# Lapis-Hong/wide_deep

Hardware: NVIDIA B200
Metric: CTR examples/sec (train step) (higher is better)
Workload: dtype bf16x3 (fp32 operands split into bf16 hi+lo, 3 tensor-core products, fp32 accumulate; 2^-16)

## Files before the change

### wide_deep_b200/csrc/api.cu

```cuda
#include <stdarg.h>
#include <stdlib.h>
#include <string.h>

#include <algorithm>
#include <cmath>
#include <random>

#include "common.cuh"
#include "farmhash.cuh"
#include "sparse_dev.cuh"

namespace wd {
static thread_local char g_err[1024] = "";
void set_error(const char* fmt, ...) {
    va_list ap;
    va_start(ap, fmt);
    vsnprintf(g_err, sizeof(g_err), fmt, ap);
    va_end(ap);
}
int init_sparse_tables(WdModel* m, uint64_t seed, int random_w);
int dense_refresh_transposes(WdModel* m);
int wide_bias_grad(WdModel* m);
int metrics_setup();
int merge_sparse(WdModel* m, int which, const void* rows, const void* grads, int64_t n);
// ... 69 lines not shown
extern "C" uint64_t wd_fingerprint_cat64(uint64_t a, uint64_t b) { return wd::fingerprint_cat64(a, b); }

namespace wd { void tc_map_cache_clear(); }

extern "C" int wd_model_destroy(WdModel* m) {
    if (!m) return WD_OK;
    cudaSetDevice(m->device);
    if (m->stream) cudaStreamSynchronize(m->stream);
    tc_map_cache_clear();
    for (auto& sl : m->slots) {
        if (sl.graph) cudaGraphExecDestroy(sl.graph);
        if (sl.graph_bwd) cudaGraphExecDestroy(sl.graph_bwd);
        if (sl.ev_up) cudaEventDestroy(sl.ev_up);
        if (sl.ev_used) cudaEventDestroy(sl.ev_used);
    }
    if (m->stream_up) { cudaStreamSynchronize(m->stream_up); cudaStreamDestroy(m->stream_up); }
    for (auto& g : m->merge_graph) if (g.exec) cudaGraphExecDestroy(g.exec);
    if (m->ev_bwd_done) cudaEventDestroy(m->ev_bwd_done);
    for (void* p : m->allocs) cudaFree(p);
    if (m->h_loss_pinned) cudaFreeHost(m->h_loss_pinned);
    for (auto& e : m->timer.ev) if (e) cudaEventDestroy(e);
    if (m->shard.aux) { cudaStreamSynchronize(m->shard.aux); cudaStreamDestroy(m->shard.aux); }
    for (cudaEvent_t ev : {m->shard.ev_a, m->shard.ev_ids2, m->shard.ev_routed1, m->shard.ev_a2, m->shard.ev_aux_done}) if (ev) cudaEventDestroy(ev);
    for (int w = 0; w < 2; ++w) {
        if (m->sstream[w]) { cudaStreamSynchronize(m->sstream[w]); cudaStreamDestroy(m->sstream[w]); }
        if (m->ev_grouped[w]) cudaEventDestroy(m->ev_grouped[w]);
        if (m->ev_done[w]) cudaEventDestroy(m->ev_done[w]);
    }
    if (m->ev_ids) cudaEventDestroy(m->ev_ids);
    if (m->ev_wide_fwd) cudaEventDestroy(m->ev_wide_fwd);
    if (m->ev_wgrad_rest) cudaEventDestroy(m->ev_wgrad_rest);
    if (m->ev_head) cudaEventDestroy(m->ev_head);
    if (m->ev_dx0) cudaEventDestroy(m->ev_dx0);
    if (m->stream) cudaStreamDestroy(m->stream);
    for (size_t i = 0; i < g_extra.size(); ++i)
        if (g_extra[i].first == m) { delete g_extra[i].second; g_extra.erase(g_extra.begin() + i); break; }
    delete m;
    return WD_OK;
}

static int init_dense_slots(WdModel* m) {
    if (m->dense_count == 0) return WD_OK;
    std::vector<float> S1(m->dense_count, 0.f);
    for (size_t i = 0; i < m->dense.size(); ++i) {
        const WdOptimizer& o = (m->use_wide && i == 0) ? m->lin_opt : m->dnn_opt;
        float s1 = slot1_init(o);
        int64_t end = i + 1 < m->dense.size() ? m->dense[i + 1].off : m->dense_count;
        for (int64_t j = m->dense[i].off; j < end; ++j) S1[j] = s1;
    }
    WD_CUDA(cudaMemcpyAsync(m->d_S1, S1.data(), S1.size() * 4, cudaMemcpyHostToDevice, m->stream));
    WD_CUDA(cudaStreamSynchronize(m->stream));
    return WD_OK;
}

static int build_model(const WdPlanDesc* d, WdModel* m, WdModelExtra* x) {
    int rc;
    m->use_wide = d->model_type & 1;
    m->use_deep = (d->model_type & 2) != 0;
    m->n_cat_fields = d->n_cat_fields; m->n_dense_fields = d->n_dense_fields; m->n_columns = d->n_columns;
    const int C = d->n_columns;
    m->col_kind.assign(d->col_kind, d->col_kind + C);
    m->col_field.assign(d->col_field, d->col_field + C);
    m->col_buckets.assign(d->col_buckets, d->col_buckets + C);
    m->col_wide_base.assign(d->col_wide_base, d->col_wide_base + C);
    m->col_emb_table.assign(d->col_emb_table, d->col_emb_table + C);
    m->col_ind_off.assign(d->col_ind_off, d->col_ind_off + C);
// ... 211 lines not shown

        int hu_off = 0, did = 0;
        for (int t = 0; t < d->n_towers; ++t) {
            Tower tw{};
            tw.n_hidden = d->tower_nlayers[t]; tw.mode = d->tower_mode[t];
            std::vector<int> hu(d->hidden_units + hu_off, d->hidden_units + hu_off + tw.n_hidden);
            hu_off += tw.n_hidden;
            const std::vector<int> units = hu;
            if (m->crelu) for (int& h : hu) h *= 2;
            auto srcs = layer_sources(tw.mode, tw.n_hidden);
            for (int l = 0; l <= tw.n_hidden; ++l) {
                Layer L{};
                if ((int)srcs[l].size() > kMaxSegs) { set_error("layer with more than %d concatenated inputs", kMaxSegs); return WD_EUNSUPPORTED; }
                L.n_in_segs = (int)srcs[l].size();
                int koff = 0, klog = 0;
                for (int s = 0; s < L.n_in_segs; ++s) {
                    int src = srcs[l][s];
                    Seg sg{};
                    sg.src = src;
                    sg.width = src < 0 ? x->d0_logical : hu[src];
                    sg.width_phys = src < 0 ? d->d0_phys : pad_to(hu[src], 32);
                    sg.k_off = koff;
                    koff += sg.width_phys; klog += sg.width;
                    L.segs[s] = sg;
                }
                L.K = klog; L.K_phys = koff;
                const bool hidden = l < tw.n_hidden;
                L.N = hidden ? hu[l] : 1;
                L.N_phys = hidden ? pad_to(hu[l], 32) : 1;
                L.N_param = hidden ? units[l] : 1;
                L.t_gamma = L.t_beta = -1;
                L.h_fp32 = false;
                for (int src : srcs[tw.n_hidden]) if (src == l) L.h_fp32 = true;
                std::vector<int> idx(4, -1);
                if (hidden) {
                    {
                        const int tn = (m->gemm_engine == WD_GEMM_BF16X3 && L.N_phys % 256 == 0) ? 256 : 128;
                        const int tiles = ((L.K_phys + 127) / 128) * ((L.N_phys + tn - 1) / tn);
                        int sp = m->wgrad_splits;
                        while (sp < 32 && tiles * sp * 2 <= 148 && m->max_batch_pad / (sp * 2) >= 512) sp *= 2;
                        L.wgrad_splits = sp;
                    }
                    L.t_kernel = add_dense(L.K_phys, L.N_phys, L.wgrad_splits, 0, (int64_t)L.K_phys * L.N_phys, true);
                    L.t_bias = add_dense(1, L.N_phys, m->row_tiles, 1, L.N_phys, false);
                    if (m->crelu) m->dense[L.t_kernel].mirror_u = m->dense[L.t_bias].mirror_u = L.N_param;
                    if (m->batch_norm) {
                        L.t_gamma = add_dense(1, L.N_phys, m->row_tiles, 1, L.N_phys, false);
                        L.t_beta = add_dense(1, L.N_phys, m->row_tiles, 1, L.N_phys, false);
                    }
                    const int64_t n = (int64_t)m->max_batch_pad * L.N_phys;
                    if ((rc = dev_alloc(m, &L.H, n))) return rc;
                    if (m->batch_norm || m->dropout_rate > 0.f) { if ((rc = dev_alloc(m, &L.A, n))) return rc; } else L.A = L.H;
                    if ((rc = dev_alloc(m, &L.HT, n))) return rc;
                    if ((rc = dev_alloc(m, &L.dH, n))) return rc;
                    if ((rc = dev_alloc(m, &L.dZ, n))) return rc;
                    if ((rc = dev_alloc(m, &L.dZT, n))) return rc;
                    if (m->gemm_engine == WD_GEMM_BF16X3)
                        for (int part = 0; part < 2; ++part) {
                            if ((rc = dev_alloc(m, &L.Hs[part], n))) return rc;
                            if ((rc = dev_alloc(m, &L.dZs[part], n))) return rc;
                        }
                } else {
                    L.t_kernel = add_dense(L.K_phys, 1, m->row_tiles, 1, L.K_phys, false);
                    L.t_bias = add_dense(1, 1, m->row_tiles, 1, 4, false);
                }
                idx[WD_D_KERNEL] = L.t_kernel; idx[WD_D_BIAS] = L.t_bias; idx[WD_D_GAMMA] = L.t_gamma; idx[WD_D_BETA] = L.t_beta;
// ... 67 lines not shown
    for (auto& e : m->timer.ev) WD_CUDA(cudaEventCreate(&e));
    WD_CUDA(cudaStreamSynchronize(m->stream));
    return WD_OK;
}

extern "C" int wd_model_create(const WdPlanDesc* d, int device, WdModel** out) {
    if (!d || !out) { set_error("null argument"); return WD_EINVAL; }
    if (d->api_version != WD_API_VERSION) { set_error("plan api_version %d != library %d", d->api_version, WD_API_VERSION); return WD_EINVAL; }
    int ndev = 0;
    if (cudaGetDeviceCount(&ndev) != cudaSuccess || ndev == 0) {
        set_error("no CUDA device: libwd_b200 has no CPU fallback");
        return WD_ENODEVICE;
    }
    if (device < 0 || device >= ndev) { set_error("device %d out of range (%d devices)", device, ndev); return WD_EINVAL; }
    WD_CUDA(cudaSetDevice(device));
    WdModel* m = new WdModel();
    WdModelExtra* x = new WdModelExtra();
    g_extra.push_back({m, x});
    m->device = device;
    memset(m->timer.ev, 0, sizeof(m->timer.ev));
    cudaError_t e = cudaStreamCreateWithFlags(&m->stream, cudaStreamNonBlocking);
    if (e == cudaSuccess) e = cudaStreamCreateWithFlags(&m->stream_up, cudaStreamNonBlocking);
    for (int w = 0; w < 2; ++w) {
        if (e == cudaSuccess) e = cudaStreamCreateWithFlags(&m->sstream[w], cudaStreamNonBlocking);
        if (e == cudaSuccess) e = cudaEventCreateWithFlags(&m->ev_grouped[w], cudaEventDisableTiming);
        if (e == cudaSuccess) e = cudaEventCreateWithFlags(&m->ev_done[w], cudaEventDisableTiming);
    }
    if (e == cudaSuccess) e = cudaEventCreateWithFlags(&m->ev_ids, cudaEventDisableTiming);
    if (e == cudaSuccess) e = cudaEventCreateWithFlags(&m->ev_wide_fwd, cudaEventDisableTiming);
    if (e == cudaSuccess) e = cudaEventCreateWithFlags(&m->ev_wgrad_rest, cudaEventDisableTiming);
    if (e == cudaSuccess) e = cudaEventCreateWithFlags(&m->ev_head, cudaEventDisableTiming);
    if (e == cudaSuccess) e = cudaEventCreateWithFlags(&m->ev_dx0, cudaEventDisableTiming);
    if (e == cudaSuccess) e = cudaEventCreateWithFlags(&m->ev_bwd_done, cudaEventDisableTiming);
    if (e != cudaSuccess) { set_error("cudaStreamCreate: %s", cudaGetErrorString(e)); wd_model_destroy(m); return WD_ECUDA; }
    m->graphs_enabled = getenv("WD_NO_GRAPH") == nullptr;
    int rc = build_model(d, m, x);
    if (rc) { wd_model_destroy(m); return rc; }
    *out = m;
    return WD_OK;
}

static int init_dense(WdModel* m, WdModelExtra* x, uint64_t seed) {
    if (m->dense_count == 0) return WD_OK;
    std::vector<float> P(m->dense_count, 0.f), S1(m->dense_count, 0.f), S2(m->dense_count, 0.f);
    std::mt19937_64 rng(seed * 7919 + 17);
    std::uniform_real_distribution<float> U(-1.f, 1.f);
    for (size_t ti = 0; ti < m->towers.size(); ++ti) {
        Tower& tw = m->towers[ti];
        for (int l = 0; l <= tw.n_hidden; ++l) {
            Layer& L = tw.layers[l];
            const DenseTensor& tk = m->dense[L.t_kernel];
            const float lim = std::sqrt(6.f / (float)(L.K + L.N_param));
            for (int s = 0; s < L.n_in_segs; ++s) {
                const Seg& sg = L.segs[s];
                for (int j = 0; j < sg.width_phys; ++j) {
                    bool real = sg.src < 0 ? (x->x0_real[j] != 0) : (j < sg.width);
                    if (!real) continue;
                    float* prow = &P[tk.off + (int64_t)(sg.k_off + j) * L.N_phys];
                    for (int n = 0; n < L.N_param; ++n) {
                        prow[n] = lim * U(rng);
                        if (tk.mirror_u) prow[n + tk.mirror_u] = -prow[n];
                    }
                }
            }
            if (L.t_gamma >= 0) for (int n = 0; n < L.N; ++n) P[m->dense[L.t_gamma].off + n] = 1.f;
        }
// ... 893 lines not shown
```

### wide_deep_b200/csrc/common.cuh

```cuda
#pragma once
#include <cuda_bf16.h>
#include <cuda_runtime.h>
#include <stdint.h>
#include <stdio.h>
#include <string>
#include <vector>

#include "../../include/wd_b200.h"

namespace wd {

constexpr int kSortTile = 1024;

void set_error(const char* fmt, ...);

#define WD_CUDA(call)                                                                         \
    do {                                                                                      \
        cudaError_t e__ = (call);                                                             \
        if (e__ != cudaSuccess) {                                                             \
            wd::set_error("%s:%d %s -> %s", __FILE__, __LINE__, #call, cudaGetErrorString(e__)); \
            return WD_ECUDA;                                                                  \
        }                                                                                     \
    } while (0)

// ... 62 lines not shown
    int64_t count;
    int rows, cols;
    int64_t gpart_off;
    int gparts;
    int g_rowtiles;
    int64_t gstride;
    int64_t wt_off;
    int mirror_u;
};

struct Seg {
    int src;
    int width;
    int width_phys;
    int k_off;
};

struct Layer {
    int n_in_segs;
    Seg segs[kMaxSegs];
    int K, K_phys;
    int N, N_phys;
    int N_param;
    int t_kernel, t_bias, t_gamma, t_beta;
    int wgrad_splits;
    float* A;
    float* H;
    float* HT;
    float* dH;
    float* dZ;
    float* dZT;
    __nv_bfloat16 *Hs[2], *dZs[2];
    bool h_fp32;
    float* colpart;
};

struct Tower {
    int n_hidden;
    int mode;
    std::vector<Layer> layers;
    float* logit;
};

struct PhaseTimer {
    static constexpr int kMax = 160;
    cudaEvent_t ev[kMax];
    const char* name[kMax];
    float ms[kMax];
    int n = 0, n_last = 0;
    bool enabled = false;
};

struct BatchSlot {
    int32_t* off = nullptr;
    uint64_t* keys = nullptr;
    float *dense = nullptr, *label = nullptr, *weight = nullptr;
    DevBatch view{};
    bool has_label = false, filled = false;
    cudaEvent_t ev_up = nullptr;
    cudaEvent_t ev_used = nullptr;
    bool up_pending = false, used_recorded = false;
    cudaGraphExec_t graph = nullptr;
    DevBatch graph_view{};
    int64_t graph_launches = 0;
    int eager_steps = 0;
    cudaGraphExec_t graph_bwd = nullptr;
// ... 55 lines not shown
    uint64_t step = 0;
    cudaEvent_t ev_a = nullptr;
    cudaStream_t aux = nullptr;
    cudaEvent_t ev_ids2 = nullptr, ev_routed1 = nullptr, ev_a2 = nullptr, ev_aux_done = nullptr;
    cudaGraphExec_t graph[64] = {};
    DevBatch graph_view[64];
    int64_t graph_launches[64] = {};
    int eager_steps[64] = {};
};
constexpr int kBarriers = 8;

}

struct WdModel {
    int device = 0;
    bool use_wide = false, use_deep = false;
    int n_cat_fields = 0, n_dense_fields = 0, n_columns = 0;
    std::vector<int32_t> col_kind, col_field, col_aux_off, col_aux_n, col_norm_kind, col_emb_table, col_ind_off;
    std::vector<int64_t> col_buckets, col_wide_base;
    std::vector<float> col_norm_a, col_norm_b;
    int n_numeric = 0;
    int d0_phys = 0;
    int64_t wide_rows = 0;
    int activation = 0, batch_norm = 0;
    WdOptimizer lin_opt{}, dnn_opt{};
    int max_batch = 0, max_batch_pad = 0;
    int64_t max_nnz = 0;
    int gemm_engine = 0;

    cudaStream_t stream = nullptr;
    cudaStream_t sstream[2] = {nullptr, nullptr};
    cudaStream_t stream_up = nullptr;
    cudaEvent_t ev_ids = nullptr, ev_head = nullptr, ev_dx0 = nullptr, ev_bwd_done = nullptr, ev_wide_fwd = nullptr, ev_wgrad_rest = nullptr;
    bool sort_smem_opt_in = false;
    bool crelu = false;
    bool list_apply_fused[2] = {false, false};
    bool record_wgrad_rest = false;
    int dense_split_tensor = -1, dense_part = 0;
    cudaEvent_t ev_grouped[2] = {nullptr, nullptr}, ev_done[2] = {nullptr, nullptr};
    bool side_pending[2] = {false, false};
    bool side_active[2] = {false, false};
    bool record_dx0 = false, dx0_recorded = false;
    struct MergeGraph { cudaGraphExec_t exec = nullptr; const void* rows = nullptr; const void* grads = nullptr; int64_t n = 0; int n_lists = 0;
                        bool on_side = false; int eager = 0; int64_t launches = 0; } merge_graph[2];
    int64_t dense_exchange_max_rows = 0;
    int64_t small_base[2] = {0, 0};
    int64_t gs_count = 0, gs_emb_floats = 0;
    int64_t gs_touch_off[2] = {0, 0};
    int n_rtab = 0, n_small_tab = 0;
    int64_t* d_rtab_row_base = nullptr;
    float** d_rtab_data = nullptr;
    int32_t *d_rtab_dim = nullptr, *d_rtab_stride = nullptr;
    int64_t* d_rtab_gs_off = nullptr;
    int32_t* d_nubig[2] = {nullptr, nullptr};
    wd::ShardState shard;
    wd::DevPlan dplan{};
    std::vector<void*> allocs;
    int64_t bytes_allocated = 0;

    int32_t *d_num_field = nullptr, *d_num_norm_kind = nullptr, *d_num_x0_off = nullptr;
    float *d_num_a = nullptr, *d_num_b = nullptr;

    int32_t* d_cat_offsets = nullptr;
    uint64_t* d_cat_keys = nullptr;
    int64_t keys_cap = 0;
    float *d_dense = nullptr, *d_label = nullptr, *d_weight = nullptr;
// ... 153 lines not shown
```

### wide_deep_b200/csrc/gemm_bf16.cu

```cuda
#include <cuda.h>
#include <stdlib.h>

#include "common.cuh"
#include "gemm.cuh"
#include "tc_ptx.cuh"

namespace wd {

int tc_make_map_bf16(CUtensorMap* map, const void* ptr, int rows, int cols, int ld, int box_rows);

namespace {

__device__ __forceinline__ void sts128(uint32_t a, uint32_t x, uint32_t y, uint32_t z, uint32_t w) {
    asm volatile("st.shared.v4.b32 [%0], {%1, %2, %3, %4};" ::"r"(a), "r"(x), "r"(y), "r"(z), "r"(w) : "memory");
}
__device__ __forceinline__ uint4 lds128(uint32_t a) {
    uint4 v;
    asm volatile("ld.shared.v4.b32 {%0, %1, %2, %3}, [%4];" : "=r"(v.x), "=r"(v.y), "=r"(v.z), "=r"(v.w) : "r"(a) : "memory");
    return v;
}
__device__ __forceinline__ void sts32f(uint32_t a, float x) { asm volatile("st.shared.f32 [%0], %1;" ::"r"(a), "f"(x) : "memory"); }
__device__ __forceinline__ float4 lds128f(uint32_t a) {
    float4 v;
    asm volatile("ld.shared.v4.f32 {%0, %1, %2, %3}, [%4];" : "=f"(v.x), "=f"(v.y), "=f"(v.z), "=f"(v.w) : "r"(a) : "memory");
// ... 244 lines not shown
                            v[4 * j4] = __float_as_uint(a0); v[4 * j4 + 1] = __float_as_uint(a1); v[4 * j4 + 2] = __float_as_uint(a2); v[4 * j4 + 3] = __float_as_uint(a3);
                            h[4 * j4] = __float_as_uint(fmaf(a0, g4.x, e4.x)); h[4 * j4 + 1] = __float_as_uint(fmaf(a1, g4.y, e4.y));
                            h[4 * j4 + 2] = __float_as_uint(fmaf(a2, g4.z, e4.z)); h[4 * j4 + 3] = __float_as_uint(fmaf(a3, g4.w, e4.w));
                        }
                        if (nb + 32 > ep.n_logical) {
#pragma unroll
                            for (int j = 0; j < 32; ++j) if (nb + j >= ep.n_logical) { v[j] = 0u; h[j] = 0u; }
                        }
                    } else {
#pragma unroll
                        for (int j = 0; j < 32; ++j) {
                            const bool ok = (nb + j) < ep.n_logical;
                            const float av = ok ? act_fwd(ep.act, __uint_as_float(v[j]) + lds32f(wp + 4 * j)) : 0.f;
                            v[j] = __float_as_uint(av);
                            h[j] = __float_as_uint(ok ? fmaf(av, lds32f(wp + 4 * (32 + j)), lds32f(wp + 4 * (64 + j))) : 0.f);
                        }
                    }
                    if (!rv) {
#pragma unroll
                        for (int j = 0; j < 32; ++j) { v[j] = 0u; h[j] = 0u; }
                    }
                    if (ep.A_out != ep.H_out) store_f32(ep.A_out, ep.ldh, mw, nb, v, false);
                    if (ep.H_out) store_f32(ep.H_out, ep.ldh, mw, nb, h, false);
                    uint32_t hh[16], hl[16];
#pragma unroll
                    for (int j = 0; j < 16; ++j) {
                        const float x0 = __uint_as_float(h[2 * j]), x1 = __uint_as_float(h[2 * j + 1]);
                        const __nv_bfloat162 hp = __floats2bfloat162_rn(x0, x1);
                        const uint32_t hb = *reinterpret_cast<const uint32_t*>(&hp);
                        const __nv_bfloat162 lp = __floats2bfloat162_rn(x0 - __uint_as_float(hb << 16), x1 - __uint_as_float(hb & 0xFFFF0000u));
                        hh[j] = hb;
                        hl[j] = *reinterpret_cast<const uint32_t*>(&lp);
                    }
                    uint8_t* dh = reinterpret_cast<uint8_t*>(ep.Hs_hi + (int64_t)mw * ep.ldh + nb);
                    uint8_t* dl = reinterpret_cast<uint8_t*>(ep.Hs_lo + (int64_t)mw * ep.ldh + nb);
                    put64(hh); flush64(dh, (int64_t)ep.ldh * 2, mw, false);
                    put64(hl); flush64(dl, (int64_t)ep.ldh * 2, mw, false);
                } else {
                    store_f32(ep.C + (MODE == EPI_WGRAD ? (int64_t)z * ep.split_stride : 0), ep.ldc, mw, nb, v, MODE == EPI_STORE && ep.accumulate);
                }
            }
            if (nkb > 0) {
                asm volatile("tcgen05.fence::before_thread_sync;" ::: "memory");
                mbar_arrive(&tmem_empty[a]);
                if (ew == 0) PROBE(use == 0 ? 5 : 7);
                ++use;
            }
        }
    }
    asm volatile("tcgen05.fence::before_thread_sync;" ::: "memory");
    __syncthreads();
    if (warp == 1) asm volatile("tcgen05.dealloc.cta_group::1.sync.aligned.b32 %0, %1;" ::"r"(tmem_base), "r"((uint32_t)(2 * TBN)));
}

__device__ __forceinline__ uint32_t cluster_rank() { uint32_t r; asm volatile("mov.u32 %0, %%cluster_ctarank;" : "=r"(r)); return r; }
__device__ __forceinline__ void cluster_sync_all() {
    asm volatile("barrier.cluster.arrive.release.aligned;\n\tbarrier.cluster.wait.acquire.aligned;" ::: "memory");
}
__device__ __forceinline__ uint32_t map_to_cta(uint32_t smem_addr, uint32_t rank) {
    uint32_t r;
    asm volatile("mapa.shared::cluster.u32 %0, %1, %2;" : "=r"(r) : "r"(smem_addr), "r"(rank));
    return r;
}
__device__ __forceinline__ void mbar_wait_wd(uint64_t* bar, uint32_t parity) {
    const uint32_t a = smem_u32(bar);
    for (uint32_t spin = 0;; ++spin) {
        uint32_t ok;
        asm volatile("{\n\t.reg .pred p;\n\tmbarrier.try_wait.parity.shared::cta.b64 p, [%1], %2;\n\tselp.u32 %0, 1, 0, p;\n\t}" : "=r"(ok) : "r"(a), "r"(parity) : "memory");
        if (ok) return;
        if (spin > (1u << 27)) { printf("libwd_b200: 2-CTA GEMM barrier watchdog (block %d thread %d)\n", blockIdx.x, threadIdx.x); __trap(); }
// ... 297 lines not shown
                            v[4 * j4] = __float_as_uint(a0); v[4 * j4 + 1] = __float_as_uint(a1); v[4 * j4 + 2] = __float_as_uint(a2); v[4 * j4 + 3] = __float_as_uint(a3);
                            h[4 * j4] = __float_as_uint(fmaf(a0, g4.x, e4.x)); h[4 * j4 + 1] = __float_as_uint(fmaf(a1, g4.y, e4.y));
                            h[4 * j4 + 2] = __float_as_uint(fmaf(a2, g4.z, e4.z)); h[4 * j4 + 3] = __float_as_uint(fmaf(a3, g4.w, e4.w));
                        }
                        if (nb + 32 > ep.n_logical) {
#pragma unroll
                            for (int j = 0; j < 32; ++j) if (nb + j >= ep.n_logical) { v[j] = 0u; h[j] = 0u; }
                        }
                    } else {
#pragma unroll
                        for (int j = 0; j < 32; ++j) {
                            const bool ok = (nb + j) < ep.n_logical;
                            const float av = ok ? act_fwd(ep.act, __uint_as_float(v[j]) + lds32f(wp + 4 * j)) : 0.f;
                            v[j] = __float_as_uint(av);
                            h[j] = __float_as_uint(ok ? fmaf(av, lds32f(wp + 4 * (32 + j)), lds32f(wp + 4 * (64 + j))) : 0.f);
                        }
                    }
                    if (!rv) {
#pragma unroll
                        for (int j = 0; j < 32; ++j) { v[j] = 0u; h[j] = 0u; }
                    }
                    if (ep.A_out != ep.H_out) store_f32(ep.A_out, ep.ldh, mw, nb, v, false);
                    if (ep.H_out) store_f32(ep.H_out, ep.ldh, mw, nb, h, false);
                    uint32_t hh[16], hl[16];
#pragma unroll
                    for (int j = 0; j < 16; ++j) {
                        const float x0 = __uint_as_float(h[2 * j]), x1 = __uint_as_float(h[2 * j + 1]);
                        const __nv_bfloat162 hp = __floats2bfloat162_rn(x0, x1);
                        const uint32_t hb = *reinterpret_cast<const uint32_t*>(&hp);
                        const __nv_bfloat162 lp = __floats2bfloat162_rn(x0 - __uint_as_float(hb << 16), x1 - __uint_as_float(hb & 0xFFFF0000u));
                        hh[j] = hb;
                        hl[j] = *reinterpret_cast<const uint32_t*>(&lp);
                    }
                    uint8_t* dh = reinterpret_cast<uint8_t*>(ep.Hs_hi + (int64_t)mw * ep.ldh + nb);
                    uint8_t* dl = reinterpret_cast<uint8_t*>(ep.Hs_lo + (int64_t)mw * ep.ldh + nb);
                    put64(hh); flush64(dh, (int64_t)ep.ldh * 2, mw, false);
                    put64(hl); flush64(dl, (int64_t)ep.ldh * 2, mw, false);
                } else if (MODE == EPI_DACT) {
                    const uint32_t wp = smem_u32(epi_params + ew * 96);
                    __syncwarp();
                    sts32f(wp + 4 * lane, pg);
                    pg = qg;
                    __syncwarp();
                    float gs[32];
#pragma unroll
                    for (int j4 = 0; j4 < 8; ++j4) {
                        const float4 t = lds128f(wp + 16 * j4);
                        gs[4 * j4] = t.x; gs[4 * j4 + 1] = t.y; gs[4 * j4 + 2] = t.z; gs[4 * j4 + 3] = t.w;
                    }
                    const bool rv = m < M;
                    float av[32], dz[32];
                    take64(ar0, av);
                    take64(ar1, av + 16);
                    const bool relu = ep.act == WD_ACT_RELU;
                    float te[32];
#pragma unroll
                    for (int j = 0; j < 32; ++j) {
                        const bool ok = rv && (nb + j) < ep.n_logical;
                        const float dh = ok ? __uint_as_float(v[j]) : 0.f;
                        const float aj = ok ? av[j] : 0.f;
                        dz[j] = relu ? (aj > 0.f ? dh * gs[j] : 0.f) : dh * gs[j] * act_bwd(ep.act, aj);
                        av[j] = dh * aj * 0.99950037468777f;
                        te[j] = dh;
                    }
                    const uint32_t cs = smem_u32(colsum + ew * 384 + (c - c_beg) * 32 + lane);
                    if (ep.bn) {
                        sts32f(cs + 512, colsum32(av, lane));
                        sts32f(cs + 1024, colsum32(te, lane));
                    }
                    {
// ... 121 lines not shown
    if (N % 32 != 0 || A.n > kMaxSegs || !B_hi || !B_lo) { set_error("bf16 GEMM engine: unsupported operands"); return WD_EUNSUPPORTED; }
    static int num_sms = 0;
    if (!num_sms) cudaDeviceGetAttribute(&num_sms, cudaDevAttrMultiProcessorCount, m->device);
    QMaps maps;
    QSegs segs{};
    segs.n = A.n;
    int rc, ktot = 0;
    const bool a_mn = mode == EPI_WGRAD, b_mn = mode == EPI_FWD || mode == EPI_WGRAD;
    for (int s = 0; s < A.n; ++s) {
        if (!A.hi[s] || !A.lo[s]) { set_error("bf16 GEMM engine: operand without hi/lo copies"); return WD_EINVAL; }
        if (!a_mn) {
            if ((rc = tc_make_map_bf16(&maps.a_hi[s], A.hi[s], M, A.k[s], A.ld[s], QBM))) return rc;
            if ((rc = tc_make_map_bf16(&maps.a_lo[s], A.lo[s], M, A.k[s], A.ld[s], QBM))) return rc;
        } else {
            if ((rc = tc_make_map_bf16(&maps.a_hi[s], A.hi[s], A.k[s], M, A.ld[s], 64))) return rc;
            if ((rc = tc_make_map_bf16(&maps.a_lo[s], A.lo[s], A.k[s], M, A.ld[s], 64))) return rc;
        }
        segs.k[s] = A.k[s]; segs.koff[s] = ktot;
        ktot += A.k[s];
    }
    for (int s = A.n; s < kMaxSegs; ++s) { maps.a_hi[s] = maps.a_hi[0]; maps.a_lo[s] = maps.a_lo[0]; }
    const bool wide = tc_bf16_wide_tile(mode, M, N, splits, num_sms);
    const bool pair = tc_bf16_uses_pair(mode, M, N, splits, num_sms);
    if (mode == EPI_DACT && !pair) { set_error("bf16 GEMM engine: the fused activation-backward epilogue exists only in the pair kernel"); return WD_EUNSUPPORTED; }
    const int tbn = wide ? 256 : 128;
    if (!b_mn) {
        if ((rc = tc_make_map_bf16(&maps.b_hi, B_hi, N, ktot, ldb, pair ? 128 : tbn))) return rc;
        if ((rc = tc_make_map_bf16(&maps.b_lo, B_lo, N, ktot, ldb, pair ? 128 : tbn))) return rc;
    } else {
        if ((rc = tc_make_map_bf16(&maps.b_hi, B_hi, ktot, N, ldb, 64))) return rc;
        if ((rc = tc_make_map_bf16(&maps.b_lo, B_lo, ktot, N, ldb, 64))) return rc;
    }
    if (mode == EPI_WGRAD) ksplit_len = (ksplit_len + QBK - 1) / QBK * QBK;
    if (mode == EPI_FWD && (!ep.Hs_hi || !ep.Hs_lo)) { set_error("bf16 GEMM engine: forward without hi/lo outputs"); return WD_EINVAL; }
#define WD_Q_LAUNCH(MODE_) \
    if (pair) return launch_pair<MODE_>(m, maps, segs, M, N, ktot, splits, ksplit_len, ep); \
    return wide ? launch_q<256, MODE_>(m, maps, segs, M, N, ktot, splits, ksplit_len, ep) : launch_q<128, MODE_>(m, maps, segs, M, N, ktot, splits, ksplit_len, ep)
    if (mode == EPI_FWD) { WD_Q_LAUNCH(EPI_FWD); }
    if (mode == EPI_STORE) { WD_Q_LAUNCH(EPI_STORE); }
    if (mode == EPI_DACT) return launch_pair<EPI_DACT>(m, maps, segs, M, N, ktot, splits, ksplit_len, ep);
    WD_Q_LAUNCH(EPI_WGRAD);
#undef WD_Q_LAUNCH
}

}
```

### wide_deep_b200/csrc/mlp.cu

```cuda
#include <stdlib.h>

#include "common.cuh"
#include "gemm.cuh"

namespace wd {

constexpr int BM = 128, BN = 128, BK = 16, GT = 256;

template <int MODE>
__global__ void __launch_bounds__(GT) gemm_tn_ffma(GemmA A, const float* __restrict__ Bm, int ldb, int M, int N, int ksplit_len, Epi ep) {
    __shared__ __align__(16) float As[2][BK][BM + 4];
    __shared__ __align__(16) float Bs[2][BK][BN + 4];
    const int tid = threadIdx.x, tx = tid & 15, ty = tid >> 4;
    const int m0 = blockIdx.y * BM, n0 = blockIdx.x * BN;
    float acc[8][8];
#pragma unroll
    for (int i = 0; i < 8; ++i)
#pragma unroll
        for (int j = 0; j < 8; ++j) acc[i][j] = 0.f;

    int ktot = 0;
    for (int s = 0; s < A.n; ++s) ktot += A.k[s];
    int kbeg = 0, kend = ktot;
    if (MODE == EPI_WGRAD) {
// ... 820 lines not shown
}

int mlp_forward(WdModel* m, bool train) {
    const int B = m->dbatch.B;
    if (!m->use_deep) return WD_OK;
    const bool q = m->gemm_engine == WD_GEMM_BF16X3;
    const __nv_bfloat16* Wq = reinterpret_cast<const __nv_bfloat16*>(m->d_Wsplit);
    if (q) {
        const int64_t n4 = (int64_t)B * m->d0_phys / 4;
        x0_split_kernel<<<grid_for(n4, 256), 256, 0, m->stream>>>(m->d_X0, n4, m->d_X0s[0], m->d_X0s[1]);
        m->launches++;
    } else if (train) {
        int Bp = (B + 127) / 128 * 128;
        dim3 g((m->d0_phys + 31) / 32, (Bp + 31) / 32);
        transpose_kernel<<<g, dim3(32, 8), 0, m->stream>>>(m->d_X0, m->d0_phys, B, Bp, m->d0_phys, m->d_X0T, m->ldt);
        m->launches++;
    }
    for (auto& tw : m->towers) {
        for (int l = 0; l < tw.n_hidden; ++l) {
            Layer& L = tw.layers[l];
            m->cur_layer = l;
            GemmA A{};
            A.n = L.n_in_segs;
            for (int s = 0; s < L.n_in_segs; ++s) {
                A.ptr[s] = src_ptr(m, tw, L.segs[s].src, false);
                A.ld[s] = src_ld(m, tw, L.segs[s].src, false);
                A.k[s] = L.segs[s].width_phys;
                if (q) { A.hi[s] = src_split(m, tw, L.segs[s].src, 0); A.lo[s] = src_split(m, tw, L.segs[s].src, 1); }
            }
            Epi ep{};
            ep.A_out = L.A; ep.H_out = L.H; ep.ldh = L.N_phys;
            ep.HT = (train && !q) ? L.HT : nullptr; ep.ldt = m->ldt;
            if (q) {
                ep.Hs_hi = L.Hs[0]; ep.Hs_lo = L.Hs[1];
                if (!L.h_fp32) ep.H_out = nullptr;
            }
            ep.bias = m->d_P + m->dense[L.t_bias].off;
            ep.gamma = L.t_gamma >= 0 ? m->d_P + m->dense[L.t_gamma].off : nullptr;
            ep.beta = L.t_beta >= 0 ? m->d_P + m->dense[L.t_beta].off : nullptr;
            ep.n_logical = L.N; ep.act = m->activation; ep.bn = m->batch_norm; ep.m_valid = B;
            const int64_t wo = m->dense[L.t_kernel].wt_off;
            const float* Wt = m->d_Wt + wo;
            int rc = run_gemm(m, EPI_FWD, A, Wt, q ? L.N_phys : L.K_phys, B, L.N_phys, ep, 1, 0, m->d_Wsplit + 2 * m->wt_count + wo,
                              m->d_Wsplit + 3 * m->wt_count + wo, Wq + wo, Wq + m->wt_count + wo);
            if (rc) return rc;
            if (train && m->dropout_rate > 0.f) {
                const DropArgs dr{m->dropout_rate, m->dropout_seed, m->d_step, (int)(&tw - &m->towers[0]) * 64 + l};
                dropout_fwd_kernel<<<grid_for((int64_t)B * L.N_phys, 256), 256, 0, m->stream>>>(B, L.N_phys, L.N, L.A, L.N_phys, ep.gamma, ep.beta, m->batch_norm,
                    (!q || L.h_fp32) ? L.H : nullptr, q ? L.Hs[0] : nullptr, q ? L.Hs[1] : nullptr, ep.HT, m->ldt, dr);
                m->launches++;
            }
        }
        Layer& LL = tw.layers[tw.n_hidden];
        GemvSegs S{};
        S.n = LL.n_in_segs;
        for (int s = 0; s < LL.n_in_segs; ++s) {
            S.ptr[s] = src_ptr(m, tw, LL.segs[s].src, false);
            S.ld[s] = src_ld(m, tw, LL.segs[s].src, false);
            S.k[s] = LL.segs[s].width_phys;
            S.koff[s] = LL.segs[s].k_off;
        }
        if ((int)m->towers.size() <= kFusedTowers) continue;
        logits_fwd_kernel<<<grid_for((int64_t)B * 32, 256), 256, 0, m->stream>>>(S, m->d_P + m->dense[LL.t_kernel].off,
                                                                                m->d_P + m->dense[LL.t_bias].off, B, tw.logit);
        m->launches++;
    }
    WD_CUDA(cudaGetLastError());
// ... 23 lines not shown
        const int blocks = grid_for((int64_t)B * 8, 256, 512);
        logits_head_kernel<<<blocks, 256, 0, m->stream>>>(in, B, m->use_wide ? m->d_wide_logit : nullptr, m->batch_has_label ? m->d_label : nullptr,
                                                         m->dbatch.weight, m->d_logits, need_grad ? m->d_dlogit : nullptr, m->d_loss_part,
                                                         m->d_head_counter, m->d_loss);
        m->launches++;
        WD_CUDA(cudaGetLastError());
        return WD_OK;
    }
    TowerLogits T{};
    T.n = m->use_deep ? (int)m->towers.size() : 0;
    for (int t = 0; t < T.n; ++t) T.p[t] = m->towers[t].logit;
    int blocks = grid_for(B, 256, 256);
    head_kernel<<<blocks, 256, 0, m->stream>>>(B, m->use_wide ? m->d_wide_logit : nullptr, T, m->batch_has_label ? m->d_label : nullptr,
                                              m->dbatch.weight, m->d_logits, need_grad ? m->d_dlogit : nullptr, m->d_loss_part);
    loss_final_kernel<<<1, 32, 0, m->stream>>>(m->d_loss_part, blocks, m->d_loss);
    m->launches += 2;
    WD_CUDA(cudaGetLastError());
    return WD_OK;
}

int mlp_backward(WdModel* m) {
    const int B = m->dbatch.B;
    if (!m->use_deep) return WD_OK;
    const int rts = (B + 127) / 128;
    const int Bk = (B + 15) / 16 * 16;
    bool dx0_written = false;
    const bool need_dx0 = !m->tables.empty();
    const bool q = m->gemm_engine == WD_GEMM_BF16X3;
    const __nv_bfloat16* Wq = reinterpret_cast<const __nv_bfloat16*>(m->d_Wsplit);
    static const bool fuse_dact_on = getenv("WD_FUSE_DACT") ? atoi(getenv("WD_FUSE_DACT")) != 0 : false;
    static const bool fuse_logits_on = getenv("WD_FUSE_LOGITS_BWD") ? atoi(getenv("WD_FUSE_LOGITS_BWD")) != 0 : true;
    static int num_sms = 0;
    if (!num_sms) cudaDeviceGetAttribute(&num_sms, cudaDevAttrMultiProcessorCount, m->device);
    for (auto& tw : m->towers) {
        std::vector<char> written(tw.n_hidden, 0);
        std::vector<int> readers(tw.n_hidden, 0);
        std::vector<char> fused(tw.n_hidden, 0);
        for (int l = 0; l <= tw.n_hidden; ++l)
            for (int s = 0; s < tw.layers[l].n_in_segs; ++s)
                if (tw.layers[l].segs[s].src >= 0) readers[tw.layers[l].segs[s].src] += (l == tw.n_hidden ? 2 : 1);
        auto grad_dst = [&](int src, float** p, int* ld, int* acc) {
            if (src < 0) { *p = m->d_dX0; *ld = m->d0_phys; *acc = dx0_written ? 1 : 0; dx0_written = true; }
            else { *p = tw.layers[src].dH; *ld = tw.layers[src].N_phys; *acc = written[src] ? 1 : 0; written[src] = 1; }
        };
        Layer& LL = tw.layers[tw.n_hidden];
        const DenseTensor& tk = m->dense[LL.t_kernel];
        const DenseTensor& tb = m->dense[LL.t_bias];
        for (int s = 0; s < LL.n_in_segs; ++s) {
            const Seg& sg = LL.segs[s];
            const float* src = src_ptr(m, tw, sg.src, false);
            int ld = src_ld(m, tw, sg.src, false);
            dim3 g((sg.width_phys + 63) / 64, rts);
            float* dst = nullptr; int dld = 0, acc = 0;
            if (!(sg.src < 0 && !need_dx0)) grad_dst(sg.src, &dst, &dld, &acc);
            const bool wb = m->use_wide && s == 0 && &tw == &m->towers.front();
            if (q && fuse_logits_on && LL.n_in_segs == 1 && sg.src >= 0 && readers[sg.src] == 2 && m->dropout_rate <= 0.f &&
                sg.width_phys == tw.layers[sg.src].N_phys) {
                Layer& S = tw.layers[sg.src];
                logits_act_bwd_q_kernel<<<dim3((S.N_phys + 63) / 64, rts), 256, 0, m->stream>>>(B, S.N_phys, S.N, src, ld, S.A, S.N_phys, m->d_dlogit,
                    m->d_P + tk.off + sg.k_off, S.t_gamma >= 0 ? m->d_P + m->dense[S.t_gamma].off : nullptr, m->activation, m->batch_norm,
                    m->d_gpart + tk.gpart_off + sg.k_off, tk.gstride, m->d_gpart + tb.gpart_off, tb.gstride,
                    wb ? m->d_gpart + m->dense[0].gpart_off : nullptr, wb ? m->dense[0].gstride : 0,
                    m->d_gpart + m->dense[S.t_bias].gpart_off, S.t_gamma >= 0 ? m->d_gpart + m->dense[S.t_gamma].gpart_off : nullptr,
                    S.t_beta >= 0 ? m->d_gpart + m->dense[S.t_beta].gpart_off : nullptr, m->dense[S.t_bias].gstride, S.dZs[0], S.dZs[1]);
                m->launches++;
                fused[sg.src] = 1;
                continue;
            }
            logits_bwd_kernel<<<g, 256, 0, m->stream>>>(B, sg.width_phys, src, ld, m->d_dlogit, m->d_P + tk.off + sg.k_off,
                                                       m->d_gpart + tk.gpart_off + sg.k_off, tk.gstride,
                                                       s == 0 ? m->d_gpart + tb.gpart_off : nullptr, tb.gstride,
                                                       wb ? m->d_gpart + m->dense[0].gpart_off : nullptr, wb ? m->dense[0].gstride : 0, dst, dld, acc);
            m->launches++;
        }
        for (int l = tw.n_hidden - 1; l >= 0; --l) {
            Layer& L = tw.layers[l];
            m->cur_layer = l;
            const DenseTensor& tkn = m->dense[L.t_kernel];
            float* pb = m->d_gpart + m->dense[L.t_bias].gpart_off;
            float* pg = L.t_gamma >= 0 ? m->d_gpart + m->dense[L.t_gamma].gpart_off : nullptr;
            float* pbe = L.t_beta >= 0 ? m->d_gpart + m->dense[L.t_beta].gpart_off : nullptr;
            if (!written[l] && !fused[l]) {
                WD_CUDA(cudaMemsetAsync(L.dH, 0, (size_t)m->max_batch_pad * L.N_phys * sizeof(float), m->stream));
            }
            dim3 g((L.N_phys + 31) / 32, rts);
            const DropArgs dr{m->dropout_rate, m->dropout_seed, m->d_step, (int)(&tw - &m->towers[0]) * 64 + l};
            if (fused[l]) {
            } else if (q)
                act_bn_bwd_q_kernel<<<dim3((L.N_phys + 63) / 64, rts), 256, 0, m->stream>>>(B, L.N_phys, L.N, L.dH, L.A, L.N_phys,
                    L.t_gamma >= 0 ? m->d_P + m->dense[L.t_gamma].off : nullptr, m->activation, m->batch_norm, pb, pg, pbe,
                    m->dense[L.t_bias].gstride, L.dZs[0], L.dZs[1], dr);
            else
            act_bn_bwd_kernel<<<g, 256, 0, m->stream>>>(B, L.N_phys, L.N, L.dH, L.A, L.N_phys,
                                                       L.t_gamma >= 0 ? m->d_P + m->dense[L.t_gamma].off : nullptr, m->activation,
                                                       m->batch_norm, L.dZ, L.dZT, m->ldt, pb, pg, pbe, m->dense[L.t_bias].gstride,
                                                       q ? L.dZs[0] : nullptr, q ? L.dZs[1] : nullptr, dr);
            if (!fused[l]) m->launches++;
            for (int s = 0; s < L.n_in_segs; ++s) {
                const Seg& sg = L.segs[s];
                if (sg.src < 0 && !need_dx0) continue;
                float* dst; int dld, acc;
                grad_dst(sg.src, &dst, &dld, &acc);
                GemmA A2{};
                A2.n = 1; A2.ptr[0] = L.dZ; A2.ld[0] = L.N_phys; A2.k[0] = L.N_phys;
                A2.hi[0] = L.dZs[0]; A2.lo[0] = L.dZs[1];
                Epi e2{};
                e2.C = dst; e2.ldc = dld; e2.accumulate = acc;
                int mode2 = EPI_STORE;
                if (q && fuse_dact_on && sg.src >= 0 && readers[sg.src] == 1 && m->dropout_rate <= 0.f && sg.width_phys == tw.layers[sg.src].N_phys &&
                    tc_bf16_uses_pair(EPI_DACT, B, sg.width_phys, 1, num_sms)) {
                    Layer& S = tw.layers[sg.src];
                    mode2 = EPI_DACT;
                    fused[sg.src] = 1;
                    e2.Aact = S.A; e2.ldh = S.N_phys; e2.Hs_hi = S.dZs[0]; e2.Hs_lo = S.dZs[1];
                    e2.gamma = S.t_gamma >= 0 ? m->d_P + m->dense[S.t_gamma].off : nullptr;
                    e2.n_logical = S.N; e2.act = m->activation; e2.bn = m->batch_norm;
                    e2.p_bias = m->d_gpart + m->dense[S.t_bias].gpart_off;
                    e2.p_gamma = S.t_gamma >= 0 ? m->d_gpart + m->dense[S.t_gamma].gpart_off : nullptr;
                    e2.p_beta = S.t_beta >= 0 ? m->d_gpart + m->dense[S.t_beta].gpart_off : nullptr;
                    e2.pstride = m->dense[S.t_bias].gstride;
                }
                const int64_t woff = tkn.wt_off + (int64_t)sg.k_off * L.N_phys;
                int rc = run_gemm(m, mode2, A2, m->d_P + tkn.off + (int64_t)sg.k_off * L.N_phys, L.N_phys, B, sg.width_phys, e2, 1, 0,
                                  m->d_Wsplit + woff, m->d_Wsplit + m->wt_count + woff, Wq + woff, Wq + m->wt_count + woff);
                if (rc) return rc;
            }
            if (l == 0 && &tw == &m->towers.back() && need_dx0 && m->ev_dx0 && m->record_dx0) {
                WD_CUDA(cudaEventRecord(m->ev_dx0, m->stream));
                m->dx0_recorded = true;
            }
        }
        for (int l = tw.n_hidden - 1; l >= 0; --l) {
            Layer& L = tw.layers[l];
            m->cur_layer = l;
            const DenseTensor& tkn = m->dense[L.t_kernel];
            if (l == 0 && m->record_wgrad_rest && m->towers.size() == 1 && L.n_in_segs == 1) {
                WD_CUDA(cudaEventRecord(m->ev_wgrad_rest, m->stream));
                m->dense_split_tensor = L.t_kernel;
            }
            for (int s = 0; s < L.n_in_segs; ++s) {
                const Seg& sg = L.segs[s];
                GemmA A{};
                A.n = 1; A.ptr[0] = src_ptr(m, tw, sg.src, true); A.ld[0] = m->ldt; A.k[0] = Bk;
                if (q) {
                    A.hi[0] = src_split(m, tw, sg.src, 0); A.lo[0] = src_split(m, tw, sg.src, 1);
                    A.ld[0] = src_ld(m, tw, sg.src, false); A.k[0] = B;
                }
                Epi ep{};
                ep.C = m->d_gpart + tkn.gpart_off + (int64_t)sg.k_off * L.N_phys; ep.ldc = L.N_phys; ep.split_stride = tkn.gstride;
                int ks = ((Bk + L.wgrad_splits - 1) / L.wgrad_splits + 31) / 32 * 32;
                if (q) ks = (ks + 63) / 64 * 64;
                int rc = run_gemm(m, EPI_WGRAD, A, L.dZT, q ? L.N_phys : m->ldt, sg.width_phys, L.N_phys, ep, L.wgrad_splits, ks, nullptr, nullptr,
                                  L.dZs[0], L.dZs[1]);
                if (rc) return rc;
            }
        }
    }
    WD_CUDA(cudaGetLastError());
    return WD_OK;
}

__global__ void crelu_fold_kernel(float* __restrict__ gp, int parts, int64_t gstride, int rows, int cols, int u) {
    const int64_t total = (int64_t)parts * rows * u;
    for (int64_t i = (int64_t)blockIdx.x * blockDim.x + threadIdx.x; i < total; i += (int64_t)gridDim.x * blockDim.x) {
        const int n = (int)(i % u);
        const int64_t pr = i / u;
        float* q = gp + (pr / rows) * gstride + (pr % rows) * cols + n;
        q[0] -= q[u];
        q[u] = 0.f;
    }
}
__global__ void crelu_mirror_kernel(float* __restrict__ P, float* __restrict__ S1, float* __restrict__ S2, int rows, int cols, int u) {
    const int64_t total = (int64_t)rows * u;
    for (int64_t i = (int64_t)blockIdx.x * blockDim.x + threadIdx.x; i < total; i += (int64_t)gridDim.x * blockDim.x) {
        const int64_t e = (i / u) * cols + i % u;
        P[e + u] = -P[e];
        S1[e + u] = S1[e];
        S2[e + u] = S2[e];
    }
}
static int crelu_fold(WdModel* m) {
    const int rts = (m->dbatch.B + 127) / 128;
    for (const DenseTensor& t : m->dense) {
        if (!t.mirror_u) continue;
        const int parts = t.g_rowtiles ? rts : t.gparts;
        crelu_fold_kernel<<<grid_for((int64_t)parts * t.rows * t.mirror_u, 256), 256, 0, m->stream>>>(m->d_gpart + t.gpart_off, parts, t.gstride, t.rows, t.cols,
                                                                                                    t.mirror_u);
        m->launches++;
// ... 74 lines not shown
```

Before: 17.59 million.

## Overlap weight-gradient GEMMs on a side stream and skip unused bf16 split stores

Weight-gradient GEMMs for hidden layers above the first are now launched on a separate stream right after each layer's dZ is ready, so they can overlap with the data-gradient chain on the main stream. The main stream joins them with an event before the remaining layer-0 wgrad. The forward epilogue also skips writing the bf16 hi/lo split of activations when no later hidden layer reads them through the GEMM, cutting store traffic. Risks include contention for SMs between the concurrent GEMMs, and a stale split buffer if some other consumer such as wgrad's src_split still reads Hs.

Measured after the change: 17.03 million, median of 6. -3.1%, worse.

```diff
diff --git a/wide_deep_b200/csrc/api.cu b/wide_deep_b200/csrc/api.cu
--- a/wide_deep_b200/csrc/api.cu
+++ b/wide_deep_b200/csrc/api.cu
@@ -125,6 +125,9 @@
     if (m->ev_wgrad_rest) cudaEventDestroy(m->ev_wgrad_rest);
     if (m->ev_head) cudaEventDestroy(m->ev_head);
     if (m->ev_dx0) cudaEventDestroy(m->ev_dx0);
+    if (m->wstream) { cudaStreamSynchronize(m->wstream); cudaStreamDestroy(m->wstream); }
+    if (m->ev_dz) cudaEventDestroy(m->ev_dz);
+    if (m->ev_wgrad_side) cudaEventDestroy(m->ev_wgrad_side);
     if (m->stream) cudaStreamDestroy(m->stream);
     for (size_t i = 0; i < g_extra.size(); ++i)
         if (g_extra[i].first == m) { delete g_extra[i].second; g_extra.erase(g_extra.begin() + i); break; }
@@ -402,6 +405,9 @@
                 L.t_gamma = L.t_beta = -1;
                 L.h_fp32 = false;
                 for (int src : srcs[tw.n_hidden]) if (src == l) L.h_fp32 = true;
+                L.gemm_read = false;
+                for (int c = l + 1; c < tw.n_hidden; ++c)
+                    for (int src : srcs[c]) if (src == l) L.gemm_read = true;
                 std::vector<int> idx(4, -1);
                 if (hidden) {
                     {
@@ -535,6 +541,9 @@
     if (e == cudaSuccess) e = cudaEventCreateWithFlags(&m->ev_head, cudaEventDisableTiming);
     if (e == cudaSuccess) e = cudaEventCreateWithFlags(&m->ev_dx0, cudaEventDisableTiming);
     if (e == cudaSuccess) e = cudaEventCreateWithFlags(&m->ev_bwd_done, cudaEventDisableTiming);
+    if (e == cudaSuccess) e = cudaStreamCreateWithFlags(&m->wstream, cudaStreamNonBlocking);
+    if (e == cudaSuccess) e = cudaEventCreateWithFlags(&m->ev_dz, cudaEventDisableTiming);
+    if (e == cudaSuccess) e = cudaEventCreateWithFlags(&m->ev_wgrad_side, cudaEventDisableTiming);
     if (e != cudaSuccess) { set_error("cudaStreamCreate: %s", cudaGetErrorString(e)); wd_model_destroy(m); return WD_ECUDA; }
     m->graphs_enabled = getenv("WD_NO_GRAPH") == nullptr;
     int rc = build_model(d, m, x);
diff --git a/wide_deep_b200/csrc/common.cuh b/wide_deep_b200/csrc/common.cuh
--- a/wide_deep_b200/csrc/common.cuh
+++ b/wide_deep_b200/csrc/common.cuh
@@ -118,6 +118,7 @@
     float* dZT;
     __nv_bfloat16 *Hs[2], *dZs[2];
     bool h_fp32;
+    bool gemm_read;
     float* colpart;
 };
 
@@ -239,6 +240,8 @@
     cudaStream_t sstream[2] = {nullptr, nullptr};
     cudaStream_t stream_up = nullptr;
     cudaEvent_t ev_ids = nullptr, ev_head = nullptr, ev_dx0 = nullptr, ev_bwd_done = nullptr, ev_wide_fwd = nullptr, ev_wgrad_rest = nullptr;
+    cudaStream_t wstream = nullptr;
+    cudaEvent_t ev_dz = nullptr, ev_wgrad_side = nullptr;
     bool sort_smem_opt_in = false;
     bool crelu = false;
     bool list_apply_fused[2] = {false, false};
diff --git a/wide_deep_b200/csrc/gemm_bf16.cu b/wide_deep_b200/csrc/gemm_bf16.cu
--- a/wide_deep_b200/csrc/gemm_bf16.cu
+++ b/wide_deep_b200/csrc/gemm_bf16.cu
@@ -300,10 +300,12 @@
                         hh[j] = hb;
                         hl[j] = *reinterpret_cast<const uint32_t*>(&lp);
                     }
-                    uint8_t* dh = reinterpret_cast<uint8_t*>(ep.Hs_hi + (int64_t)mw * ep.ldh + nb);
-                    uint8_t* dl = reinterpret_cast<uint8_t*>(ep.Hs_lo + (int64_t)mw * ep.ldh + nb);
-                    put64(hh); flush64(dh, (int64_t)ep.ldh * 2, mw, false);
-                    put64(hl); flush64(dl, (int64_t)ep.ldh * 2, mw, false);
+                    if (ep.Hs_hi) {
+                        uint8_t* dh = reinterpret_cast<uint8_t*>(ep.Hs_hi + (int64_t)mw * ep.ldh + nb);
+                        uint8_t* dl = reinterpret_cast<uint8_t*>(ep.Hs_lo + (int64_t)mw * ep.ldh + nb);
+                        put64(hh); flush64(dh, (int64_t)ep.ldh * 2, mw, false);
+                        put64(hl); flush64(dl, (int64_t)ep.ldh * 2, mw, false);
+                    }
                 } else {
                     store_f32(ep.C + (MODE == EPI_WGRAD ? (int64_t)z * ep.split_stride : 0), ep.ldc, mw, nb, v, MODE == EPI_STORE && ep.accumulate);
                 }
@@ -667,10 +669,12 @@
                         hh[j] = hb;
                         hl[j] = *reinterpret_cast<const uint32_t*>(&lp);
                     }
-                    uint8_t* dh = reinterpret_cast<uint8_t*>(ep.Hs_hi + (int64_t)mw * ep.ldh + nb);
-                    uint8_t* dl = reinterpret_cast<uint8_t*>(ep.Hs_lo + (int64_t)mw * ep.ldh + nb);
-                    put64(hh); flush64(dh, (int64_t)ep.ldh * 2, mw, false);
-                    put64(hl); flush64(dl, (int64_t)ep.ldh * 2, mw, false);
+                    if (ep.Hs_hi) {
+                        uint8_t* dh = reinterpret_cast<uint8_t*>(ep.Hs_hi + (int64_t)mw * ep.ldh + nb);
+                        uint8_t* dl = reinterpret_cast<uint8_t*>(ep.Hs_lo + (int64_t)mw * ep.ldh + nb);
+                        put64(hh); flush64(dh, (int64_t)ep.ldh * 2, mw, false);
+                        put64(hl); flush64(dl, (int64_t)ep.ldh * 2, mw, false);
+                    }
                 } else if (MODE == EPI_DACT) {
                     const uint32_t wp = smem_u32(epi_params + ew * 96);
                     __syncwarp();
@@ -858,7 +862,7 @@
         if ((rc = tc_make_map_bf16(&maps.b_lo, B_lo, ktot, N, ldb, 64))) return rc;
     }
     if (mode == EPI_WGRAD) ksplit_len = (ksplit_len + QBK - 1) / QBK * QBK;
-    if (mode == EPI_FWD && (!ep.Hs_hi || !ep.Hs_lo)) { set_error("bf16 GEMM engine: forward without hi/lo outputs"); return WD_EINVAL; }
+    if (mode == EPI_FWD && !ep.Hs_hi && !ep.H_out) { set_error("bf16 GEMM engine: forward without outputs"); return WD_EINVAL; }
 #define WD_Q_LAUNCH(MODE_) \
     if (pair) return launch_pair<MODE_>(m, maps, segs, M, N, ktot, splits, ksplit_len, ep); \
     return wide ? launch_q<256, MODE_>(m, maps, segs, M, N, ktot, splits, ksplit_len, ep) : launch_q<128, MODE_>(m, maps, segs, M, N, ktot, splits, ksplit_len, ep)
diff --git a/wide_deep_b200/csrc/mlp.cu b/wide_deep_b200/csrc/mlp.cu
--- a/wide_deep_b200/csrc/mlp.cu
+++ b/wide_deep_b200/csrc/mlp.cu
@@ -876,7 +876,7 @@
             ep.A_out = L.A; ep.H_out = L.H; ep.ldh = L.N_phys;
             ep.HT = (train && !q) ? L.HT : nullptr; ep.ldt = m->ldt;
             if (q) {
-                ep.Hs_hi = L.Hs[0]; ep.Hs_lo = L.Hs[1];
+                if (L.gemm_read) { ep.Hs_hi = L.Hs[0]; ep.Hs_lo = L.Hs[1]; }
                 if (!L.h_fp32) ep.H_out = nullptr;
             }
             ep.bias = m->d_P + m->dense[L.t_bias].off;
@@ -966,6 +966,7 @@
     static const bool fuse_logits_on = getenv("WD_FUSE_LOGITS_BWD") ? atoi(getenv("WD_FUSE_LOGITS_BWD")) != 0 : true;
     static int num_sms = 0;
     if (!num_sms) cudaDeviceGetAttribute(&num_sms, cudaDevAttrMultiProcessorCount, m->device);
+    const bool side_wgrad = q && !m->timer.enabled;
     for (auto& tw : m->towers) {
         std::vector<char> written(tw.n_hidden, 0);
         std::vector<int> readers(tw.n_hidden, 0);
@@ -973,6 +974,29 @@
         for (int l = 0; l <= tw.n_hidden; ++l)
             for (int s = 0; s < tw.layers[l].n_in_segs; ++s)
                 if (tw.layers[l].segs[s].src >= 0) readers[tw.layers[l].segs[s].src] += (l == tw.n_hidden ? 2 : 1);
+        auto wgrad = [&](int l) -> int {
+            Layer& L = tw.layers[l];
+            m->cur_layer = l;
+            const DenseTensor& tkn = m->dense[L.t_kernel];
+            for (int s = 0; s < L.n_in_segs; ++s) {
+                const Seg& sg = L.segs[s];
+                GemmA A{};
+                A.n = 1; A.ptr[0] = src_ptr(m, tw, sg.src, true); A.ld[0] = m->ldt; A.k[0] = Bk;
+                if (q) {
+                    A.hi[0] = src_split(m, tw, sg.src, 0); A.lo[0] = src_split(m, tw, sg.src, 1);
+                    A.ld[0] = src_ld(m, tw, sg.src, false); A.k[0] = B;
+                }
+                Epi ep{};
+                ep.C = m->d_gpart + tkn.gpart_off + (int64_t)sg.k_off * L.N_phys; ep.ldc = L.N_phys; ep.split_stride = tkn.gstride;
+                int ks = ((Bk + L.wgrad_splits - 1) / L.wgrad_splits + 31) / 32 * 32;
+                if (q) ks = (ks + 63) / 64 * 64;
+                int rc = run_gemm(m, EPI_WGRAD, A, L.dZT, q ? L.N_phys : m->ldt, sg.width_phys, L.N_phys, ep, L.wgrad_splits, ks, nullptr, nullptr,
+                                  L.dZs[0], L.dZs[1]);
+                if (rc) return rc;
+            }
+            return WD_OK;
+        };
+        bool side_used = false;
         auto grad_dst = [&](int src, float** p, int* ld, int* acc) {
             if (src < 0) { *p = m->d_dX0; *ld = m->d0_phys; *acc = dx0_written ? 1 : 0; dx0_written = true; }
             else { *p = tw.layers[src].dH; *ld = tw.layers[src].N_phys; *acc = written[src] ? 1 : 0; written[src] = 1; }
@@ -1030,6 +1054,16 @@
                                                        m->batch_norm, L.dZ, L.dZT, m->ldt, pb, pg, pbe, m->dense[L.t_bias].gstride,
                                                        q ? L.dZs[0] : nullptr, q ? L.dZs[1] : nullptr, dr);
             if (!fused[l]) m->launches++;
+            if (side_wgrad && l >= 1) {
+                WD_CUDA(cudaEventRecord(m->ev_dz, m->stream));
+                WD_CUDA(cudaStreamWaitEvent(m->wstream, m->ev_dz, 0));
+                cudaStream_t main_stream = m->stream;
+                m->stream = m->wstream;
+                int rc = wgrad(l);
+                m->stream = main_stream;
+                if (rc) return rc;
+                side_used = true;
+            }
             for (int s = 0; s < L.n_in_segs; ++s) {
                 const Seg& sg = L.segs[s];
                 if (sg.src < 0 && !need_dx0) continue;
@@ -1064,30 +1098,19 @@
                 m->dx0_recorded = true;
             }
         }
+        if (side_used) {
+            WD_CUDA(cudaEventRecord(m->ev_wgrad_side, m->wstream));
+            WD_CUDA(cudaStreamWaitEvent(m->stream, m->ev_wgrad_side, 0));
+        }
         for (int l = tw.n_hidden - 1; l >= 0; --l) {
+            if (side_wgrad && l >= 1) continue;
             Layer& L = tw.layers[l];
-            m->cur_layer = l;
-            const DenseTensor& tkn = m->dense[L.t_kernel];
             if (l == 0 && m->record_wgrad_rest && m->towers.size() == 1 && L.n_in_segs == 1) {
                 WD_CUDA(cudaEventRecord(m->ev_wgrad_rest, m->stream));
                 m->dense_split_tensor = L.t_kernel;
             }
-            for (int s = 0; s < L.n_in_segs; ++s) {
-                const Seg& sg = L.segs[s];
-                GemmA A{};
-                A.n = 1; A.ptr[0] = src_ptr(m, tw, sg.src, true); A.ld[0] = m->ldt; A.k[0] = Bk;
-                if (q) {
-                    A.hi[0] = src_split(m, tw, sg.src, 0); A.lo[0] = src_split(m, tw, sg.src, 1);
-                    A.ld[0] = src_ld(m, tw, sg.src, false); A.k[0] = B;
-                }
-                Epi ep{};
-                ep.C = m->d_gpart + tkn.gpart_off + (int64_t)sg.k_off * L.N_phys; ep.ldc = L.N_phys; ep.split_stride = tkn.gstride;
-                int ks = ((Bk + L.wgrad_splits - 1) / L.wgrad_splits + 31) / 32 * 32;
-                if (q) ks = (ks + 63) / 64 * 64;
-                int rc = run_gemm(m, EPI_WGRAD, A, L.dZT, q ? L.N_phys : m->ldt, sg.width_phys, L.N_phys, ep, L.wgrad_splits, ks, nullptr, nullptr,
-                                  L.dZs[0], L.dZs[1]);
-                if (rc) return rc;
-            }
+            int rc = wgrad(l);
+            if (rc) return rc;
         }
     }
     WD_CUDA(cudaGetLastError());
```
